# openhumanoids/pronto

Measured on NVIDIA B200. Metric: rbis_ekf_filter_steps_per_s, higher is better.
Workload: dtype f64

## Files before the change

### dev/kbench.cu

```cuda
#include <cuda_runtime.h>
#include <cmath>
#include <cstdio>
#include <cstdlib>
#include <cstring>
#include <vector>
#include <string>

#define CK(x) do { cudaError_t e = (x); if (e != cudaSuccess) { printf("CUDA error %s at %s:%d\n", cudaGetErrorString(e), __FILE__, __LINE__); exit(1); } } while (0)

struct Variant {
  const char* name;
  int tpb;
  int smem;
  void (*geom)(long long N, int sms, int* grid, int* tpb, int* smem);
  void (*launch)(void* kparams_blob, int grid, int tpb, int smem, cudaStream_t st);
  size_t kparams_size;
  void (*fill)(void* blob, long long N, double* vec, double* quat, double* P, double* ll, double* q4, const double* imu,
               const void* ops, long long n_ops, const double* z0, const double* z1, const double* q1, const double* R0,
               const double* R1);
  void (*prep)(int smem);
};
std::vector<Variant>& registry() { static std::vector<Variant> r; return r; }

__global__ void __launch_bounds__(256) dfma_probe(double* out, int iters, double a, int active_lanes) {
// ... 89 lines not shown
        double v = (i == j) ? 0.01 * (1 + 0.1 * rnd()) : 1e-4 * rnd();
        if (decoupled && (passive(i) || passive(j)) && !blk) v = 0.0;
        P[(size_t)(j * (j + 1) / 2 + i) * N + n] = v;
      }
    q4[n] = 7.6e-5; q4[N + n] = 1e-2; q4[2 * N + n] = 3e-10; q4[3 * N + n] = 1e-6;
    for (int i = 0; i < pi; i++) for (int c = 0; c < 4; c++) q1[((size_t)i * 4 + c) * N + n] = quat[c * N + n];
  }
  for (auto& v : imu) v = 0.05 * rnd();
  for (long long k = 0; k < T; k++) for (long long n = 0; n < N; n++) imu[(k * 6 + 5) * N + n] += 9.8;
  for (auto& v : z0) v = 0.1 * rnd();
  for (auto& v : z1) v = 0.1 * rnd();
  double R0[9] = {0.01, 0, 0, 0, 0.01, 0, 0, 0, 0.01};
  double R1[36] = {0};
  for (int i = 0; i < 6; i++) R1[i * 7] = i < 3 ? 0.0025 : 0.0012;
  double *d_vec, *d_quat, *d_P, *d_ll, *d_q4, *d_imu, *d_z0, *d_z1, *d_q1, *d_R0, *d_R1;
  void* d_ops;
  CK(cudaMalloc(&d_vec, vec.size() * 8)); CK(cudaMalloc(&d_quat, quat.size() * 8)); CK(cudaMalloc(&d_P, P.size() * 8));
  CK(cudaMalloc(&d_ll, N * 8)); CK(cudaMalloc(&d_q4, q4.size() * 8)); CK(cudaMalloc(&d_imu, imu.size() * 8));
  CK(cudaMalloc(&d_z0, z0.size() * 8)); CK(cudaMalloc(&d_z1, z1.size() * 8)); CK(cudaMalloc(&d_q1, q1.size() * 8));
  CK(cudaMalloc(&d_R0, 81 * 8)); CK(cudaMalloc(&d_R1, 81 * 8)); CK(cudaMalloc(&d_ops, ops.size() * sizeof(Op)));
  CK(cudaMemcpy(d_q4, q4.data(), q4.size() * 8, cudaMemcpyHostToDevice));
  CK(cudaMemcpy(d_imu, imu.data(), imu.size() * 8, cudaMemcpyHostToDevice));
  CK(cudaMemcpy(d_z0, z0.data(), z0.size() * 8, cudaMemcpyHostToDevice));
  CK(cudaMemcpy(d_z1, z1.data(), z1.size() * 8, cudaMemcpyHostToDevice));
  CK(cudaMemcpy(d_q1, q1.data(), q1.size() * 8, cudaMemcpyHostToDevice));
  CK(cudaMemcpy(d_R0, R0, 72, cudaMemcpyHostToDevice)); CK(cudaMemcpy(d_R1, R1, 36 * 8, cudaMemcpyHostToDevice));
  CK(cudaMemcpy(d_ops, ops.data(), ops.size() * sizeof(Op), cudaMemcpyHostToDevice));
  std::vector<double> ref_vec, ref_P, out_vec(vec.size()), out_P(P.size());
  for (auto& v : registry()) {
    if (only && !strstr(v.name, only)) continue;
    std::vector<char> blob(v.kparams_size, 0);
    int grid, tpb, smem;
    v.geom(N, prop.multiProcessorCount, &grid, &tpb, &smem);
    v.prep(smem);
    float best = 1e30f;
    for (int rep = 0; rep < 3; rep++) {
      CK(cudaMemcpy(d_vec, vec.data(), vec.size() * 8, cudaMemcpyHostToDevice));
      CK(cudaMemcpy(d_quat, quat.data(), quat.size() * 8, cudaMemcpyHostToDevice));
      CK(cudaMemcpy(d_P, P.data(), P.size() * 8, cudaMemcpyHostToDevice));
      CK(cudaMemset(d_ll, 0, N * 8));
      v.fill(blob.data(), N, d_vec, d_quat, d_P, d_ll, d_q4, d_imu, d_ops, (long long)ops.size(), d_z0, d_z1, d_q1, d_R0, d_R1);
      CK(cudaEventRecord(e0));
      v.launch(blob.data(), grid, tpb, smem, 0);
      CK(cudaEventRecord(e1)); CK(cudaEventSynchronize(e1)); CK(cudaGetLastError());
      CK(cudaEventElapsedTime(&ms, e0, e1));
      if (ms < best) best = ms;
    }
    CK(cudaMemcpy(out_vec.data(), d_vec, vec.size() * 8, cudaMemcpyDeviceToHost));
    CK(cudaMemcpy(out_P.data(), d_P, P.size() * 8, cudaMemcpyDeviceToHost));
    double ev = 0, eP = 0;
    if (ref_vec.empty()) { ref_vec = out_vec; ref_P = out_P; }
    for (size_t i = 0; i < out_vec.size(); i++) ev = fmax(ev, fabs(out_vec[i] - ref_vec[i]) / fmax(1.0, fabs(ref_vec[i])));
    for (size_t i = 0; i < out_P.size(); i++) eP = fmax(eP, fabs(out_P[i] - ref_P[i]) / 0.01);
    bool finite = true;
    for (size_t i = 0; i < out_vec.size(); i++) if (!std::isfinite(out_vec[i])) finite = false;
    printf("%-28s grid %4d x %3d thr, %6d B smem: %8.3f ms  %7.3f G filter-steps/s  (vs first: dvec %.2e dP %.2e finite=%d)\n", v.name, grid, tpb, smem, best,
// ... 5 lines not shown
```

### dev/kvariant.cu

```cuda
#include <cuda_runtime.h>
#include <cstring>
#include <vector>
#define rbisk VNAME
#ifdef KV1
#define KFUNC rbis_fused_kernel
#define SET_FAST(s, c, v)
#else
#ifdef KGROUP
#ifndef KDC
#define KDC 0
#endif
#ifndef KMAXW
#define KMAXW 8
#endif
#define KFUNC grp::rbis_group_kernel<KGROUP, (KDC != 0), KMAXW>
#elif defined(KDC)
#define KFUNC rbis_fused_kernel<false, true>
#else
#define KFUNC rbis_fused_kernel<false>
#endif
#define SET_FAST(s, c, v) s.chunk_fast[c] = v
#endif
#ifndef KHEADER
#define KHEADER "../pronto_b200/csrc/rbis_kernels.cuh"
// ... 35 lines not shown
  *smem = wpc * GE::FPW * GE::S * 8;
}
#else
void geom(long long N, int, int* grid, int* tpb, int* smem) {
  *tpb = VNAME::TPB; *smem = VNAME::SMEM_BYTES; *grid = (int)((N + VNAME::TPB - 1) / VNAME::TPB);
}
#endif
void prep(int smem) { cudaFuncSetAttribute(VNAME::KFUNC, cudaFuncAttributeMaxDynamicSharedMemorySize, smem); }
void fill(void* blob, long long N, double* vec, double* quat, double* P, double* ll, double* q4, const double* imu,
          const void* ops, long long n_ops, const double* z0, const double* z1, const double* q1, const double* R0,
          const double* R1) {
  VNAME::KParams kp;
  std::memset(&kp, 0, sizeof(kp));
  kp.N = N; kp.vec = vec; kp.quat = quat; kp.P = P; kp.loglik = ll;
  kp.q_gyro = q4; kp.q_accel = q4 + N; kp.q_gyro_bias = q4 + 2 * N; kp.q_accel_bias = q4 + 3 * N;
  kp.imu = imu; kp.imu_cols = N; kp.ops = (const VNAME::Op*)ops; kp.n_ops = n_ops; kp.g_val = 9.8; kp.chi_tol = 1e-6; kp.ctor_folds_chi = 1;
  auto& s0 = kp.streams[0];
  s0.m = 3; s0.has_orient = 0; s0.r_mode = 0; s0.n_chunks = 1; s0.idx[0] = 3; s0.idx[1] = 4; s0.idx[2] = 5;
  s0.chunk_start[0] = 0; s0.chunk_len[0] = 3; SET_FAST(s0, 0, 3); s0.z = z0; s0.R = R0; s0.cols = N;
  auto& s1 = kp.streams[1];
  s1.m = 6; s1.has_orient = 1; s1.r_mode = 0; s1.n_chunks = 2;
  int idx[6] = {9, 10, 11, 6, 7, 8};
  for (int i = 0; i < 6; i++) s1.idx[i] = idx[i];
  s1.chunk_start[0] = 0; s1.chunk_len[0] = 3; s1.chunk_start[1] = 3; s1.chunk_len[1] = 3; SET_FAST(s1, 0, 9); SET_FAST(s1, 1, 6); s1.z = z1; s1.quat = q1; s1.R = R1; s1.cols = N;
  std::memcpy(blob, &kp, sizeof(kp));
}
struct Reg { Reg() { registry().push_back({VTAG, VNAME::TPB, VNAME::SMEM_BYTES, geom, launch, sizeof(VNAME::KParams), fill, prep}); } } reg;
}
```

### include/rbis_batch.h

```cpp
#ifndef RBIS_BATCH_H_
#define RBIS_BATCH_H_

#include <stdint.h>

#ifdef __cplusplus
extern "C" {
#endif

#define RBIS_NUM_STATES 21
#define RBIS_COV_ELEMS 441
#define RBIS_MAX_MEAS 9
#define RBIS_MAX_STREAMS 8
#define RBIS_NUM_STATS 96

typedef struct rbis_batch rbis_batch_t;

typedef enum {
  RBIS_OK = 0,
  RBIS_ERR_INVALID = -1,
  RBIS_ERR_CUDA = -2,
  RBIS_ERR_ALLOC = -3,
  RBIS_ERR_STATE = -4
} rbis_status_t;

// ... 96 lines not shown
  int32_t cov_blocks;
} rbis_record_t;
int rbis_batch_set_record(rbis_batch_t* h, const rbis_record_t* rec);

#define RBIS_INNOV_NIS    1
#define RBIS_INNOV_Y      2
#define RBIS_INNOV_S_DIAG 4
typedef struct {
  uint32_t fields;
  int32_t  m;
  double*  out;
  int64_t  rows;
} rbis_innovation_t;
int rbis_batch_set_innovations(rbis_batch_t* h, int32_t stream, const rbis_innovation_t* spec);

int rbis_batch_run_fused(rbis_batch_t* h, int64_t n_ops, const rbis_op_t* ops, const double* imu,
                         int64_t imu_rows, int n_streams, const rbis_stream_t* streams, int mem);

typedef struct {
  int32_t m;
  int32_t has_orientation;
  int32_t channel;
  int32_t channel_rot;
  const double* mean;
  const double* mean_quat;
  const int64_t* step;
  double sigma[RBIS_MAX_MEAS];
  double sigma_rot[3];
  int64_t rows;
} rbis_synth_stream_t;
typedef struct {
  uint64_t seed;
// ... 114 lines not shown
```

### pronto_b200/capi.py

```python
import ctypes as C
import os

_HERE = os.path.dirname(os.path.abspath(__file__))
LIB_PATH = os.path.join(_HERE, "lib", "librbis_b200.so")

NUM_STATES = 21
COV_ELEMS = 441
MAX_MEAS = 9
MAX_STREAMS = 8
NUM_STATS = 96

MEM_HOST, MEM_DEVICE = 0, 1
MEM_F32_ROWS = 4
OP_IMU, OP_MEAS, OP_SNAPSHOT, OP_RESTORE, OP_RECORD = 0, 1, 2, 3, 4
REC_FIELDS = 47
REC_BLOCKS = 7
INNOV_NIS, INNOV_Y, INNOV_S_DIAG = 1, 2, 4
R_SHARED_FULL, R_PER_FILTER_DIAG, R_PER_ROW_FULL = 0, 1, 2
STREAM_SKIP_NAN_ROWS = 1

c_double_p = C.POINTER(C.c_double)
c_int32_p = C.POINTER(C.c_int32)
c_int64_p = C.POINTER(C.c_int64)


class Config(C.Structure):
    _fields_ = [
        ("g_val", C.c_double),
        ("chi_tol", C.c_double),
# ... 106 lines not shown
    ]


PROTOTYPES = {
    "rbis_last_error": (C.c_char_p, []),
    "rbis_default_config": (None, [C.POINTER(Config)]),
    "rbis_batch_create": (C.c_int, [C.POINTER(C.c_void_p), C.c_int64, C.POINTER(Config)]),
    "rbis_batch_destroy": (C.c_int, [C.c_void_p]),
    "rbis_batch_synchronize": (C.c_int, [C.c_void_p]),
    "rbis_batch_num_filters": (C.c_int64, [C.c_void_p]),
    "rbis_batch_stream": (C.c_void_p, [C.c_void_p]),
    "rbis_batch_launch_count": (C.c_int64, [C.c_void_p]),
    "rbis_batch_last_kernel_variant": (C.c_int, [C.c_void_p]),
    "rbis_batch_notch_configure": (C.c_int, [C.c_void_p, C.c_double, C.c_double, C.c_int, C.c_int64]),
    "rbis_batch_notch_filter": (C.c_int, [C.c_void_p, C.c_void_p, C.c_int64, C.c_int]),
    "rbis_smooth_plan": (C.c_int64, [C.c_int64, C.c_void_p, C.c_void_p, C.c_void_p, C.c_void_p, C.c_void_p, C.c_void_p]),
    "rbis_batch_smooth_backward": (C.c_int, [C.c_void_p, C.c_int32, C.c_int32, C.c_int64, C.c_void_p, C.c_double]),
    "rbis_batch_get_snapshot": (C.c_int, [C.c_void_p, C.c_int32, C.c_void_p, C.c_void_p, C.c_void_p, C.c_void_p, C.c_int]),
    "rbis_batch_set_state": (C.c_int, [C.c_void_p, C.c_void_p, C.c_void_p, C.c_void_p, C.c_void_p, C.c_int64, C.c_int]),
    "rbis_batch_get_state": (C.c_int, [C.c_void_p, C.c_void_p, C.c_void_p, C.c_void_p, C.c_void_p, c_int64_p, C.c_int]),
    "rbis_batch_set_filter": (C.c_int, [C.c_void_p, C.c_int64, C.c_void_p, C.c_void_p, C.c_void_p, C.c_double]),
    "rbis_batch_get_filter": (C.c_int, [C.c_void_p, C.c_int64, C.c_void_p, C.c_void_p, C.c_void_p, c_double_p]),
    "rbis_batch_set_process_noise": (C.c_int, [C.c_void_p, C.c_double, C.c_double, C.c_double, C.c_double]),
    "rbis_batch_set_process_noise_per_filter": (C.c_int, [C.c_void_p, C.c_void_p, C.c_void_p, C.c_void_p, C.c_void_p, C.c_int]),
    "rbis_batch_ins_step": (C.c_int, [C.c_void_p, C.c_void_p, C.c_void_p, C.c_double, C.c_int64, C.c_int]),
    "rbis_batch_indexed_update": (C.c_int, [C.c_void_p, C.c_int, c_int32_p, C.c_void_p, C.c_void_p, C.c_int, C.c_int64, C.c_int]),
    "rbis_batch_indexed_orient_update": (C.c_int, [C.c_void_p, C.c_int, c_int32_p, C.c_void_p, C.c_void_p, C.c_void_p, C.c_int, C.c_int64, C.c_int]),
    "rbis_batch_set_column_map": (C.c_int, [C.c_void_p, C.c_int, C.c_void_p, C.c_int64]),
    "rbis_batch_set_record": (C.c_int, [C.c_void_p, C.POINTER(Record)]),
    "rbis_batch_set_innovations": (C.c_int, [C.c_void_p, C.c_int32, C.POINTER(Innovation)]),
# ... 65 lines not shown
```

### pronto_b200/csrc/rbis_batch.cu

```cuda
#include <cuda_runtime.h>
#include <dlfcn.h>

#include <algorithm>
#include <cmath>
#include <cstdarg>
#include <cstdio>
#include <cstring>
#include <new>
#include <string>
#include <vector>

#include "../../include/rbis_batch.h"
#include "rbis_kernels.cuh"
#include "rbis_stats.cuh"
#include "rbis_smooth.cuh"
#include "rbis_synth.cuh"
#include "rbis_fused_tu.h"

namespace {

thread_local std::string g_last_error;

int fail(int code, const char* fmt, ...) {
  char buf[512];
// ... 71 lines not shown
  int* d_flag = nullptr;
  rbisk::NotchCoeffs notch{};
  double* d_notch_state = nullptr;
  int64_t notch_cols = 0;
  DevBuf notch_stage;
  int last_variant = -1;
  int mapping = 1;
  int lane_tpb = 384;
  int n_sms = 148;
  long long last_part = -1;
  DevBuf full_cov;
  DevBuf misc;
  DevBuf stats_async;
  DevBuf synth_small;
  DevBuf stats_table;
  rbisk::Op* d_ops = nullptr;
  size_t d_ops_cap = 0;
  double* d_rshared = nullptr;
  StagingSlot slots[2];
  int slot_toggle = 0;
  int* d_map[1 + RBIS_MAX_STREAMS] = {};
  int64_t map_cols[1 + RBIS_MAX_STREAMS] = {};
  static constexpr int kMaxGroups = 8, kRing = 8;
  int n_groups = 1;
  cudaStream_t gstream[kMaxGroups] = {};
  cudaStream_t upload_stream = nullptr;
  cudaEvent_t gdone[kRing][kMaxGroups] = {};
  bool gdone_valid[kRing] = {};
  cudaEvent_t uploaded[kRing] = {};
  cudaEvent_t pre_evt = nullptr;
  cudaEvent_t syn_evt = nullptr;
  static constexpr int kPinSlots = 16;
  static constexpr size_t kPinBytes = 128 << 10;
  char* pin_base = nullptr;
  cudaEvent_t pin_evt[kPinSlots] = {};
  int pin_next = 0;
  DevBuf d_syn;
  DevBuf d_syn_ring[kRing];
  rbisk::Op* d_ops_ring[kRing] = {};
  size_t d_ops_ring_cap[kRing] = {};
  double* d_rshared_ring[kRing] = {};
  int64_t launch_seq = 0;
  int last_ring = -1;
  bool groups_dirty = false;
  bool stream_dirty = true;
  cudaEvent_t tickets[8] = {};
  int next_ticket = 0;
  bool rec_set = false;
  rbis_record_t rec{};
  int rec_k = 0;
  cudaStream_t rec_stream = nullptr;
  cudaEvent_t rec_launched = nullptr;
  DevBuf rec_stage[2];
  cudaEvent_t rec_copied[2] = {};
  bool rec_pending[2] = {};
// ... 177 lines not shown
  auto aligned_triple = [&](int a) {
    return d.idx[a] % 3 == 0 && d.idx[a + 1] == d.idx[a] + 1 && d.idx[a + 2] == d.idx[a] + 2;
  };
  for (size_t i = 0; i + 1 < cut.size();) {
    const int a = cut[i], blen = cut[i + 1] - cut[i];
    if (blen == 1 && i + 3 < cut.size() && cut[i + 2] - cut[i + 1] == 1 && cut[i + 3] - cut[i + 2] == 1 && aligned_triple(a)) {
      d.chunk_start[d.n_chunks] = a;
      d.chunk_len[d.n_chunks++] = 3;
      i += 3;
      continue;
    }
    d.chunk_start[d.n_chunks] = a;
    d.chunk_len[d.n_chunks++] = blen;
    i += 1;
  }
}

int upload_small(rbis_batch* h, void* dst, const void* src, size_t bytes, cudaStream_t st) {
  if (bytes == 0) return 0;
  if (!h->pin_base || bytes > rbis_batch::kPinBytes) {
    CUDA_TRY(cudaMemcpyAsync(dst, src, bytes, cudaMemcpyHostToDevice, st));
    return 0;
  }
  const int k = h->pin_next;
  h->pin_next = (k + 1) % rbis_batch::kPinSlots;
  CUDA_TRY(cudaEventSynchronize(h->pin_evt[k]));
  char* p = h->pin_base + (size_t)k * rbis_batch::kPinBytes;
  std::memcpy(p, src, bytes);
  CUDA_TRY(cudaMemcpyAsync(dst, p, bytes, cudaMemcpyHostToDevice, st));
  CUDA_TRY(cudaEventRecord(h->pin_evt[k], st));
// ... 218 lines not shown
      case RBIS_OP_RESTORE:
        if (o.row < 0 || o.row >= h->cfg.snapshot_slots) return fail(RBIS_ERR_INVALID, "op %lld: snapshot slot %lld out of range (%d slots)", (long long)i, (long long)o.row, h->cfg.snapshot_slots);
        if (!snap_valid[(size_t)o.row]) return fail(RBIS_ERR_STATE, "op %lld: restore of empty snapshot slot %lld", (long long)i, (long long)o.row);
        if (!snap_dc[(size_t)o.row]) restores_ok = false;
        last_utime = o.utime;
        break;
      case RBIS_OP_RECORD:
        if (!h->rec_set) return fail(RBIS_ERR_STATE, "op %lld: RBIS_OP_RECORD but no record set (rbis_batch_set_record)", (long long)i);
        if (o.row < 0 || o.row >= h->rec.rows) return fail(RBIS_ERR_INVALID, "op %lld: record row %lld out of range (%lld rows)", (long long)i, (long long)o.row, (long long)h->rec.rows);
        rec_rows.push_back(o.row);
        any_record = true;
        break;
      default:
        return fail(RBIS_ERR_INVALID, "op %lld: unknown kind %d", (long long)i, o.kind);
    }
  }

  rbisk::KParams kp;
  std::memset(&kp, 0, sizeof(kp));
  kp.N = N;
  kp.vec = h->vec; kp.quat = h->quat; kp.P = h->P; kp.loglik = h->loglik;
  kp.q_gyro = h->qparams; kp.q_accel = h->qparams + N; kp.q_gyro_bias = h->qparams + 2 * N;
  kp.q_accel_bias = h->qparams + 3 * N;
  kp.snap = h->snap;
  kp.n_snap = h->cfg.snapshot_slots;
  kp.n_ops = n_ops;
  kp.g_val = h->cfg.g_val; kp.chi_tol = h->cfg.chi_tol;
  kp.ctor_folds_chi = h->cfg.ctor_folds_chi; kp.renorm = h->cfg.renormalize_quat;

  kp.imu_map = use_maps ? h->d_map[0] : nullptr;
// ... 229 lines not shown
  if (any_snapshot && !h->snap_read_pending.empty()) {
    for (int64_t i = 0; i < n_ops; i++)
      if (ops[i].kind == RBIS_OP_SNAPSHOT && h->snap_read_pending[(size_t)ops[i].row]) {
        slot_readers.push_back(h->snap_read_evt[(size_t)ops[i].row]);
        h->snap_read_pending[(size_t)ops[i].row] = 0;
      }
  }
  if (any_record && !rec_host) take_readers(h, h->rec.out, h->rec.out + (size_t)h->rec.rows * (size_t)h->rec_k * N, slot_readers);
  for (int s = 0; s < n_streams; s++)
    if (innov_used[s]) take_readers(h, h->innov[s].out, h->innov[s].out + (size_t)h->innov[s].rows * (size_t)h->innov_k[s] * N, slot_readers);
  if (!grouped) {
    if (int rc = main_stream_work(h)) return rc;
    for (cudaEvent_t e : slot_readers) CUDA_TRY(cudaStreamWaitEvent(h->stream, e, 0));
    if (staging) CUDA_TRY(cudaStreamWaitEvent(h->stream, slot.copied, 0));
    if (rec_host && h->rec_pending[rec_b]) CUDA_TRY(cudaStreamWaitEvent(h->stream, h->rec_copied[rec_b], 0));
    if ((size_t)n_ops > h->d_ops_cap) {
      if (h->d_ops) {
        CUDA_TRY(cudaStreamSynchronize(h->stream));
        cudaFree(h->d_ops);
        h->d_ops = nullptr;
        h->d_ops_cap = 0;
      }
      size_t cap = (size_t)n_ops * 2;
      if (cap < 1024) cap = 1024;
      CUDA_TRY(cudaMalloc(&h->d_ops, cap * sizeof(rbisk::Op)));
      h->d_ops_cap = cap;
    }
    if (int rc = upload_small(h, h->d_ops, kops.data(), (size_t)n_ops * sizeof(rbisk::Op), h->stream)) return rc;
    if (any_shared)
      if (int rc = upload_small(h, h->d_rshared, rshared.data(), rshared.size() * sizeof(double), h->stream)) return rc;
    if (fuse_syn) {
      if (h->d_syn.cap < syn_host.size()) {
        CUDA_TRY(cudaStreamSynchronize(h->stream));
        if (h->d_syn.ensure(syn_host.size() * 2)) return fail(RBIS_ERR_ALLOC, "synth row buffer allocation failed");
      }
      if (int rc = upload_small(h, h->d_syn.p, syn_host.data(), syn_host.size() * 8, h->stream)) return rc;
      point_syn(h->d_syn.p);
    }
    kp.ops = h->d_ops;
    kp.block_offset = 0;
    CUDA_TRY(launch_variant(variant, fuse_syn ? 1 : 0, geom, grid, h->stream, kp));
    h->launches++;
    if (staging) CUDA_TRY(cudaEventRecord(slot.consumed, h->stream));
    if (rec_host) {
      CUDA_TRY(cudaEventRecord(h->rec_launched, h->stream));
      CUDA_TRY(cudaStreamWaitEvent(h->rec_stream, h->rec_launched, 0));
    }
  } else {
    const int64_t piece_ops = h->cfg.piece_ops > 0 ? h->cfg.piece_ops : 256;
    const int64_t pieces = n_ops >= 2 * piece_ops ? (n_ops + piece_ops - 1) / piece_ops : 1;
    const unsigned per = (grid + (unsigned)h->n_groups - 1) / (unsigned)h->n_groups;
    const long long part = (long long)per * geom.fpc;
    for (int64_t pc = 0; pc < pieces; pc++) {
      const int64_t o0 = n_ops * pc / pieces, o1 = n_ops * (pc + 1) / pieces, np = o1 - o0;
      const int ring = (int)(h->launch_seq % rbis_batch::kRing);
      if (h->gdone_valid[ring])
        for (int g = 0; g < h->n_groups; g++) CUDA_TRY(cudaEventSynchronize(h->gdone[ring][g]));
      if ((size_t)np > h->d_ops_ring_cap[ring]) {
        if (h->d_ops_ring[ring]) cudaFree(h->d_ops_ring[ring]);
        h->d_ops_ring[ring] = nullptr;
        h->d_ops_ring_cap[ring] = 0;
        size_t cap = (size_t)np * 2;
        if (cap < 1024) cap = 1024;
        CUDA_TRY(cudaMalloc(&h->d_ops_ring[ring], cap * sizeof(rbisk::Op)));
        h->d_ops_ring_cap[ring] = cap;
      }
      if (int rc = upload_small(h, h->d_ops_ring[ring], kops.data() + o0, (size_t)np * sizeof(rbisk::Op), h->upload_stream)) return rc;
      if (any_shared) {
        if (int rc = upload_small(h, h->d_rshared_ring[ring], rshared.data(), rshared.size() * sizeof(double), h->upload_stream)) return rc;
        for (int s2 = 0; s2 < n_streams; s2++)
          if (shared_r[s2]) kp.streams[s2].R = h->d_rshared_ring[ring] + (size_t)s2 * kRShared;
      }
      if (fuse_syn) {
        if (h->d_syn_ring[ring].cap < syn_host.size() && h->d_syn_ring[ring].ensure(syn_host.size() * 2))
          return fail(RBIS_ERR_ALLOC, "synth row buffer allocation failed");
        if (int rc = upload_small(h, h->d_syn_ring[ring].p, syn_host.data(), syn_host.size() * 8, h->upload_stream)) return rc;
        point_syn(h->d_syn_ring[ring].p);
      }
      CUDA_TRY(cudaEventRecord(h->uploaded[ring], h->upload_stream));
      kp.ops = h->d_ops_ring[ring];
      kp.n_ops = np;
      const bool wait_main = h->stream_dirty;
      if (wait_main) CUDA_TRY(cudaEventRecord(h->pre_evt, h->stream));
      const bool repartitioned = h->last_ring >= 0 && h->groups_dirty && h->last_part != part;
      for (int g = 0; g < h->n_groups; g++) {
        const unsigned b0 = (unsigned)g * per, b1 = b0 + per < grid ? b0 + per : grid;
        cudaStream_t gs = h->gstream[g];
        if (repartitioned)
          for (int g2 = 0; g2 < h->n_groups; g2++) CUDA_TRY(cudaStreamWaitEvent(gs, h->gdone[h->last_ring][g2], 0));
        if (wait_main) CUDA_TRY(cudaStreamWaitEvent(gs, h->pre_evt, 0));
        if (pc == 0)
          for (cudaEvent_t e : slot_readers) CUDA_TRY(cudaStreamWaitEvent(gs, e, 0));
        if (staging && pc == 0) CUDA_TRY(cudaStreamWaitEvent(gs, slot.copied, 0));
        if (rec_host && pc == 0 && h->rec_pending[rec_b]) CUDA_TRY(cudaStreamWaitEvent(gs, h->rec_copied[rec_b], 0));
        CUDA_TRY(cudaStreamWaitEvent(gs, h->uploaded[ring], 0));
        if (b1 > b0) {
          kp.block_offset = (int)b0;
          CUDA_TRY(launch_variant(variant, fuse_syn ? 1 : 0, geom, b1 - b0, gs, kp));
          h->launches++;
        }
        CUDA_TRY(cudaEventRecord(h->gdone[ring][g], gs));
      }
      h->gdone_valid[ring] = true;
      h->last_ring = ring;
      h->last_part = part;
      h->groups_dirty = true;
      h->stream_dirty = false;
      if (staging) slot.ring = ring;
      if (pc + 1 < pieces) h->launch_seq++;
    }
    if (rec_host)
      for (int g = 0; g < h->n_groups; g++) CUDA_TRY(cudaStreamWaitEvent(h->rec_stream, h->gdone[h->last_ring][g], 0));
  }
  if (rec_host) {
    const size_t row_doubles = (size_t)h->rec_k * (size_t)N;
    for (size_t a = 0; a < rec_distinct.size();) {
      size_t e = a + 1;
      while (e < rec_distinct.size() && rec_distinct[e] == rec_distinct[e - 1] + 1) e++;
      CUDA_TRY(cudaMemcpyAsync(h->rec.out + (size_t)rec_distinct[a] * row_doubles, h->rec_stage[rec_b].p + a * row_doubles,
                               (e - a) * row_doubles * sizeof(double), cudaMemcpyDeviceToHost, h->rec_stream));
      a = e;
    }
    CUDA_TRY(cudaEventRecord(h->rec_copied[rec_b], h->rec_stream));
    h->rec_pending[rec_b] = true;
// ... 10 lines not shown
    const char as_launch = ((variant & 2) || (before == 1 && !passive_index && restores_ok)) ? 1 : 0;
    for (auto& f : snap_dc)
      if (f == 2) f = as_launch;
  }
  h->snap_dc = snap_dc;
  h->last_variant = variant | (fuse_syn ? 4 : 0) | (h->mapping > 1 ? (h->mapping << 4) : 0);
  h->utime = last_utime;
  return 0;
}

}

extern "C" {

const char* rbis_last_error(void) { return g_last_error.c_str(); }

void rbis_default_config(rbis_batch_config_t* cfg) {
  if (!cfg) return;
  cfg->g_val = 9.8;
  cfg->chi_tol = 1e-6;
  cfg->ctor_folds_chi = 1;
  cfg->renormalize_quat = 0;
  cfg->snapshot_slots = 0;
  cfg->device = 0;
  cfg->launch_groups = 0;
  cfg->dense_only = 0;
  cfg->mapping = 0;
  cfg->lane_filters_per_cta = 0;
  cfg->piece_ops = 0;
  cfg->synth_materialize = 0;
// ... 118 lines not shown
  if (h->copy_stream) cudaStreamSynchronize(h->copy_stream);
  if (h->rec_stream) { cudaStreamSynchronize(h->rec_stream); cudaStreamDestroy(h->rec_stream); }
  if (h->rec_launched) cudaEventDestroy(h->rec_launched);
  for (auto& e : h->rec_copied)
    if (e) cudaEventDestroy(e);
  for (auto& e : h->ticket_rec)
    if (e) cudaEventDestroy(e);
  for (auto& b : h->rec_stage) b.release();
  if (h->upload_stream) { cudaStreamSynchronize(h->upload_stream); cudaStreamDestroy(h->upload_stream); }
  for (int g = 0; g < rbis_batch::kMaxGroups; g++)
    if (h->gstream[g]) { cudaStreamSynchronize(h->gstream[g]); cudaStreamDestroy(h->gstream[g]); }
  for (int r = 0; r < rbis_batch::kRing; r++) {
    if (h->uploaded[r]) cudaEventDestroy(h->uploaded[r]);
    for (int g = 0; g < rbis_batch::kMaxGroups; g++)
      if (h->gdone[r][g]) cudaEventDestroy(h->gdone[r][g]);
    cudaFree(h->d_ops_ring[r]);
    cudaFree(h->d_rshared_ring[r]);
  }
  if (h->pre_evt) cudaEventDestroy(h->pre_evt);
  if (h->syn_evt) cudaEventDestroy(h->syn_evt);
  for (auto& e : h->pin_evt)
    if (e) cudaEventDestroy(e);
  if (h->pin_base) cudaFreeHost(h->pin_base);
  cudaFree(h->vec); cudaFree(h->quat); cudaFree(h->P); cudaFree(h->loglik); cudaFree(h->qparams);
  cudaFree(h->snap); cudaFree(h->d_ops); cudaFree(h->d_rshared); cudaFree(h->d_flag); cudaFree(h->d_notch_state);
  h->notch_stage.release();
  for (auto& m : h->d_map) cudaFree(m);
  h->full_cov.release(); h->misc.release(); h->stats_async.release(); h->stats_table.release(); h->synth_small.release(); h->d_syn.release();
  for (auto& b : h->snap_stats_scratch) b.release();
  for (cudaEvent_t e : h->snap_read_evt) if (e) cudaEventDestroy(e);
  for (auto& r : h->row_readers) cudaEventDestroy(r.done);
  if (h->rec_stats_done) cudaEventDestroy(h->rec_stats_done);
  h->rec_stats_scratch.release();
  if (h->stats_stream) cudaStreamDestroy(h->stats_stream);
  for (auto& b : h->d_syn_ring) b.release();
  for (auto& s : h->slots) {
    s.imu.release(); s.f32.release(); s.rtab.release();
    for (int i = 0; i < RBIS_MAX_STREAMS; i++) { s.z[i].release(); s.quat[i].release(); s.rdiag[i].release(); }
    if (s.copied) cudaEventDestroy(s.copied);
    if (s.consumed) cudaEventDestroy(s.consumed);
// ... 822 lines not shown
```

### pronto_b200/csrc/rbis_group.cuh

```cuda
#ifndef RBIS_GROUP_CUH_
#define RBIS_GROUP_CUH_

namespace rbisk {
namespace grp {

template <int G, bool DC>
struct Geo {
  static_assert(G == 2 || G == 4 || G == 8 || G == 16, "lanes per filter");
  static constexpr int NA = DC ? N_ACT : NS;
  static constexpr int LD = NA;
  static constexpr int FPW = 32 / G;
  static constexpr int NJ = (NA + G - 1) / G;
  static constexpr int stride_() {
    int s = NA * LD;
    while (s % 16 != G % 16) s++;
    return s;
  }
  static constexpr int S = stride_();
  static constexpr int PV = DC ? 0 : 3, PC = DC ? 3 : 6, PP = DC ? 6 : 9, PG = DC ? 9 : 15, PA = DC ? 12 : 18;
};
template <bool DC>
__device__ __forceinline__ int pos_of(int idx) { return DC ? (idx < 12 ? idx - 3 : idx - 6) : idx; }
template <bool DC>
__host__ __device__ constexpr int idx_of(int pos) { return DC ? act_col(pos) : pos; }
// ... 550 lines not shown
  const int wpc = blockDim.x >> 5;
  const long long N = p.N;
  long long n = (((long long)blockIdx.x + p.block_offset) * wpc + warp) * FPW + lane / G;
  const bool active = n < N;
  if (!active) n = N - 1;
  const bool writer = active && l == 0;
  double* Pf = smem + (size_t)(warp * FPW + lane / G) * S;

  FilterState s;
  static_for<NS>([&](auto i) { s.x[i] = p.vec[(long long)i * N + n]; });
  s.qw = p.quat[n]; s.qx = p.quat[N + n]; s.qy = p.quat[2 * N + n]; s.qz = p.quat[3 * N + n];
  s.ll = p.loglik[n];
  g_cov_load<G, DC>(Pf, l, p.P + n, N);
  bool imu_seen = false;

  auto load_op = [&](long long i) {
    Op o;
    long long w0, w1;
    asm volatile("ld.global.nc.s64 %0, [%1];" : "=l"(w0) : "l"(reinterpret_cast<const long long*>(p.ops + i)));
    asm volatile("ld.global.nc.s64 %0, [%1];" : "=l"(w1) : "l"(reinterpret_cast<const long long*>(p.ops + i) + 1));
    o.kind = (int)(w0 & 0xffffffffll); o.stream = (int)(w0 >> 32); o.row = w1;
    asm volatile("ld.global.nc.f64 %0, [%1];" : "=d"(o.dt) : "l"(&p.ops[i].dt));
    return o;
  };
  const long long imu_n = p.imu_map ? (long long)__ldg(p.imu_map + n) : n;
  QNoise qn;
  qn.q_gyro = __ldg(p.q_gyro + n); qn.q_accel = __ldg(p.q_accel + n);
  qn.q_gyro_bias = __ldg(p.q_gyro_bias + n); qn.q_accel_bias = __ldg(p.q_accel_bias + n);

  auto prefetch = [&](const double* ptr) { asm volatile("prefetch.global.L1 [%0];" ::"l"(ptr)); };
  unsigned long long syn_kf = 0;
  double syn_sg = 0.0, syn_sa = 0.0;
  if constexpr (SYN) {
    syn_kf = p.syn.seed ^ ((unsigned long long)(p.syn.first_filter + n) * SYN_K1);
    syn_sg = p.syn.sigma_gyro >= 0 ? p.syn.sigma_gyro : sqrt(__ldg(p.q_gyro + n) / p.syn.dt);
    syn_sa = p.syn.sigma_accel >= 0 ? p.syn.sigma_accel : sqrt(__ldg(p.q_accel + n) / p.syn.dt);
  }
  auto prefetch_inputs = [&](const Op& o) {
    if (o.kind == OP_IMU) {
      const double* base = p.imu + o.row * 6 * p.imu_cols + imu_n;
#pragma unroll
      for (int k = 0; k < 6; k++) prefetch(base + k * p.imu_cols);
    } else if (o.kind == OP_MEAS) {
      const StreamDesc& st = p.streams[o.stream];
      const long long sn = st.map ? (long long)__ldg(st.map + n) : n;
      const double* zb = st.z + o.row * st.m * st.cols + sn;
      for (int a = 0; a < st.m; a++) prefetch(zb + a * st.cols);
      if (st.has_orient) {
        const double* qb = st.quat + o.row * 4 * st.cols + sn;
#pragma unroll
        for (int k = 0; k < 4; k++) prefetch(qb + k * st.cols);
      }
    }
  };
  Op op1 = load_op(0);
  Op op2 = p.n_ops > 1 ? load_op(1) : op1;
  for (long long oi = 0; oi < p.n_ops; oi++) {
    const Op op = op1;
    op1 = op2;
    if (oi + 2 < p.n_ops) op2 = load_op(oi + 2);
    if constexpr (!SYN) {
      if (oi + 1 < p.n_ops) prefetch_inputs(op1);
    }
    if (op.kind == OP_IMU) {
      const double* base = p.imu + op.row * 6 * p.imu_cols + imu_n;
      const long long Ni = p.imu_cols;
      V3 gyro, acc;
      if constexpr (SYN) {
        const unsigned long long kfs = syn_kf ^ ((unsigned long long)__ldg(p.syn.imu_step + op.row) * SYN_K2);
        const double* mu = p.syn.imu_mean + op.row * 6;
        double nn[6];
        syn_normals_k<1, 6>(kfs, 0u, nn);
        gyro = {fma(syn_sg, nn[0], __ldg(mu)), fma(syn_sg, nn[1], __ldg(mu + 1)), fma(syn_sg, nn[2], __ldg(mu + 2))};
        acc = {fma(syn_sa, nn[3], __ldg(mu + 3)), fma(syn_sa, nn[4], __ldg(mu + 4)), fma(syn_sa, nn[5], __ldg(mu + 5))};
      } else {
        gyro = {ldg_early(base), ldg_early(base + Ni), ldg_early(base + 2 * Ni)};
        acc = {ldg_early(base + 3 * Ni), ldg_early(base + 4 * Ni), ldg_early(base + 5 * Ni)};
// ... 127 lines not shown
```

### pronto_b200/csrc/rbis_kernels.cuh

```cuda
#if defined(rbisk) || !defined(RBIS_KERNELS_CUH_DEFAULT)
#ifndef rbisk
#define RBIS_KERNELS_CUH_DEFAULT
#endif
#include <cstdint>
#include <utility>

#define RBIS_SCHED_FENCE() asm volatile("" ::: "memory")
#ifndef RBIS_LATE_LOADS
#define RBIS_LATE_LOADS 0
#endif
#ifndef RBIS_PARK_STATE
#define RBIS_PARK_STATE 0
#endif

namespace rbisk {

constexpr int NS = 21;
constexpr int NP = 231;
#ifndef RBIS_TPB
#define RBIS_TPB 256
#endif
constexpr int TPB = RBIS_TPB;
constexpr int SWEEP_TILE = 8;
constexpr int MAX_MEAS = 9;
// ... 96 lines not shown
  int chunk_fast[MAX_CHUNKS];
  const double* z;
  const double* quat;
  const double* R;
  const int* map;
  long long cols;
  long long r_stride;
};

struct Op {
  int kind, stream;
  long long row;
  double dt;
};
constexpr int OP_IMU = 0, OP_MEAS = 1, OP_SNAPSHOT = 2, OP_RECORD = 4;

constexpr unsigned long long SYN_K1 = 0x9E3779B97F4A7C15ull, SYN_K2 = 0xC2B2AE3D27D4EB4Full, SYN_K3 = 0x165667B19E3779F9ull;
__host__ __device__ __forceinline__ unsigned long long splitmix64(unsigned long long x) {
  x += 0x9E3779B97F4A7C15ull;
  x = (x ^ (x >> 30)) * 0xBF58476D1CE4E5B9ull;
  x = (x ^ (x >> 27)) * 0x94D049BB133111EBull;
  return x ^ (x >> 31);
}
struct SynPair {
  float r, th;
};
__device__ __forceinline__ SynPair syn_pair_k(unsigned long long kfs, unsigned even_channel) {
  const unsigned long long a = splitmix64(kfs ^ ((unsigned long long)even_channel * SYN_K3));
  const float u1 = ((float)(unsigned)(a >> 40) + 0.5f) * (1.0f / 16777216.0f);
  const float u2 = (float)((unsigned)(a >> 16) & 0xffffffu) * (1.0f / 16777216.0f);
// ... 83 lines not shown

struct KParams {
  long long N;
  double* vec;
  double* quat;
  double* P;
  double* loglik;
  const double* q_gyro;
  const double* q_accel;
  const double* q_gyro_bias;
  const double* q_accel_bias;
  const double* imu;
  const int* imu_map;
  long long imu_cols;
  double* snap;
  const Op* ops;
  long long n_ops;
  double g_val, chi_tol;
  int ctor_folds_chi, renorm, n_snap;
  int block_offset;
  StreamDesc streams[MAX_STREAMS];
  SynK syn;
  RecK rec;
  unsigned skip_nan_streams;
  unsigned rec_cov_blocks;
  InnovK innov[MAX_STREAMS];
};

template <int... Is, class F>
__device__ __forceinline__ void static_for_impl(std::integer_sequence<int, Is...>, F&& f) {
  (f(std::integral_constant<int, Is>{}), ...);
}
template <int N, class F>
__device__ __forceinline__ void static_for(F&& f) {
  static_for_impl(std::make_integer_sequence<int, N>{}, static_cast<F&&>(f));
}

struct V3 {
  double x, y, z;
};
__device__ __forceinline__ V3 cross(const V3& a, const V3& b) {
  return {fma(a.y, b.z, -(a.z * b.y)), fma(a.z, b.x, -(a.x * b.z)), fma(a.x, b.y, -(a.y * b.x))};
// ... 1000 lines not shown
  long long n = ((long long)blockIdx.x + p.block_offset) * TPB + tid;
  const bool active = n < N;
  if (!active) n = N - 1;

  Cov P;
  P.Ps = smem + tid;
  P.tm = tm_base + ((uint32_t)((warp & 3) * 32) << 16) + (uint32_t)((warp >> 2) * TM_COLS);
  FilterState s;
  static_for<NS>([&](auto i) { s.x[i] = p.vec[(long long)i * N + n]; });
  s.qw = p.quat[n]; s.qx = p.quat[N + n]; s.qy = p.quat[2 * N + n]; s.qz = p.quat[3 * N + n];
  s.ll = p.loglik[n];
  if constexpr (DC) cov_load_active(P, p.P + n, N);
  else cov_load_all(P, p.P + n, N);
  bool imu_seen = false;

  auto load_op = [&](long long i) {
    Op o;
    long long w0, w1;
    asm volatile("ld.global.nc.s64 %0, [%1];" : "=l"(w0) : "l"(reinterpret_cast<const long long*>(p.ops + i)));
    asm volatile("ld.global.nc.s64 %0, [%1];" : "=l"(w1) : "l"(reinterpret_cast<const long long*>(p.ops + i) + 1));
    o.kind = (int)(w0 & 0xffffffffll); o.stream = (int)(w0 >> 32); o.row = w1;
    asm volatile("ld.global.nc.f64 %0, [%1];" : "=d"(o.dt) : "l"(&p.ops[i].dt));
    return o;
  };
  const long long imu_n = p.imu_map ? (long long)__ldg(p.imu_map + n) : n;
  unsigned long long syn_kf = 0;
  double syn_sg = 0.0, syn_sa = 0.0;
  if constexpr (SYN) {
    syn_kf = p.syn.seed ^ ((unsigned long long)(p.syn.first_filter + n) * SYN_K1);
    syn_sg = p.syn.sigma_gyro >= 0 ? p.syn.sigma_gyro : sqrt(__ldg(p.q_gyro + n) / p.syn.dt);
    syn_sa = p.syn.sigma_accel >= 0 ? p.syn.sigma_accel : sqrt(__ldg(p.q_accel + n) / p.syn.dt);
  }
  Op op_next = load_op(0);
  for (long long oi = 0; oi < p.n_ops; oi++) {
    const Op op = op_next;
    if (oi + 1 < p.n_ops) op_next = load_op(oi + 1);
    if (op.kind == OP_IMU) {
      const double* base = p.imu + op.row * 6 * p.imu_cols + imu_n;
      const long long Ni = p.imu_cols;
      V3 gyro, acc;
      QNoise qn;
      auto load_q = [&]() {
        qn.q_gyro = ldg_early(p.q_gyro + n); qn.q_accel = ldg_early(p.q_accel + n);
        qn.q_gyro_bias = ldg_early(p.q_gyro_bias + n); qn.q_accel_bias = ldg_early(p.q_accel_bias + n);
      };
      auto load_inputs = [&]() {
        if constexpr (SYN) {
          const unsigned long long kfs = syn_kf ^ ((unsigned long long)__ldg(p.syn.imu_step + op.row) * SYN_K2);
          const double* mu = p.syn.imu_mean + op.row * 6;
          double nn[6];
          syn_normals_k<1, 6>(kfs, 0u, nn);
// ... 198 lines not shown
```

Baseline: 7.238 billion.

## Pass the op schedule as a packed table in kernel parameters instead of global memory

```diff
diff --git a/dev/kbench.cu b/dev/kbench.cu
--- a/dev/kbench.cu
+++ b/dev/kbench.cu
@@ -127,18 +127,16 @@
   double R1[36] = {0};
   for (int i = 0; i < 6; i++) R1[i * 7] = i < 3 ? 0.0025 : 0.0012;
   double *d_vec, *d_quat, *d_P, *d_ll, *d_q4, *d_imu, *d_z0, *d_z1, *d_q1, *d_R0, *d_R1;
-  void* d_ops;
   CK(cudaMalloc(&d_vec, vec.size() * 8)); CK(cudaMalloc(&d_quat, quat.size() * 8)); CK(cudaMalloc(&d_P, P.size() * 8));
   CK(cudaMalloc(&d_ll, N * 8)); CK(cudaMalloc(&d_q4, q4.size() * 8)); CK(cudaMalloc(&d_imu, imu.size() * 8));
   CK(cudaMalloc(&d_z0, z0.size() * 8)); CK(cudaMalloc(&d_z1, z1.size() * 8)); CK(cudaMalloc(&d_q1, q1.size() * 8));
-  CK(cudaMalloc(&d_R0, 81 * 8)); CK(cudaMalloc(&d_R1, 81 * 8)); CK(cudaMalloc(&d_ops, ops.size() * sizeof(Op)));
+  CK(cudaMalloc(&d_R0, 81 * 8)); CK(cudaMalloc(&d_R1, 81 * 8));
   CK(cudaMemcpy(d_q4, q4.data(), q4.size() * 8, cudaMemcpyHostToDevice));
   CK(cudaMemcpy(d_imu, imu.data(), imu.size() * 8, cudaMemcpyHostToDevice));
   CK(cudaMemcpy(d_z0, z0.data(), z0.size() * 8, cudaMemcpyHostToDevice));
   CK(cudaMemcpy(d_z1, z1.data(), z1.size() * 8, cudaMemcpyHostToDevice));
   CK(cudaMemcpy(d_q1, q1.data(), q1.size() * 8, cudaMemcpyHostToDevice));
   CK(cudaMemcpy(d_R0, R0, 72, cudaMemcpyHostToDevice)); CK(cudaMemcpy(d_R1, R1, 36 * 8, cudaMemcpyHostToDevice));
-  CK(cudaMemcpy(d_ops, ops.data(), ops.size() * sizeof(Op), cudaMemcpyHostToDevice));
   std::vector<double> ref_vec, ref_P, out_vec(vec.size()), out_P(P.size());
   for (auto& v : registry()) {
     if (only && !strstr(v.name, only)) continue;
@@ -152,7 +150,7 @@
       CK(cudaMemcpy(d_quat, quat.data(), quat.size() * 8, cudaMemcpyHostToDevice));
       CK(cudaMemcpy(d_P, P.data(), P.size() * 8, cudaMemcpyHostToDevice));
       CK(cudaMemset(d_ll, 0, N * 8));
-      v.fill(blob.data(), N, d_vec, d_quat, d_P, d_ll, d_q4, d_imu, d_ops, (long long)ops.size(), d_z0, d_z1, d_q1, d_R0, d_R1);
+      v.fill(blob.data(), N, d_vec, d_quat, d_P, d_ll, d_q4, d_imu, ops.data(), (long long)ops.size(), d_z0, d_z1, d_q1, d_R0, d_R1);
       CK(cudaEventRecord(e0));
       v.launch(blob.data(), grid, tpb, smem, 0);
       CK(cudaEventRecord(e1)); CK(cudaEventSynchronize(e1)); CK(cudaGetLastError());
diff --git a/dev/kvariant.cu b/dev/kvariant.cu
--- a/dev/kvariant.cu
+++ b/dev/kvariant.cu
@@ -73,7 +73,20 @@
   std::memset(&kp, 0, sizeof(kp));
   kp.N = N; kp.vec = vec; kp.quat = quat; kp.P = P; kp.loglik = ll;
   kp.q_gyro = q4; kp.q_accel = q4 + N; kp.q_gyro_bias = q4 + 2 * N; kp.q_accel_bias = q4 + 3 * N;
-  kp.imu = imu; kp.imu_cols = N; kp.ops = (const VNAME::Op*)ops; kp.n_ops = n_ops; kp.g_val = 9.8; kp.chi_tol = 1e-6; kp.ctor_folds_chi = 1;
+  kp.imu = imu; kp.imu_cols = N; kp.g_val = 9.8; kp.chi_tol = 1e-6; kp.ctor_folds_chi = 1;
+  const VNAME::Op* o = (const VNAME::Op*)ops;
+  int nd = 0;
+  long long i = 0;
+  for (; i < n_ops && i < VNAME::OPTAB_OPS; i++) {
+    int di = 0;
+    while (di < nd && std::memcmp(&kp.prog.dt[di], &o[i].dt, 8)) di++;
+    if (di == nd) {
+      if (nd == VNAME::OPTAB_DTS) break;
+      kp.prog.dt[nd++] = o[i].dt;
+    }
+    kp.prog.op[i] = VNAME::optab_word(o[i].kind, o[i].stream, (unsigned)di, (unsigned long long)o[i].row);
+  }
+  kp.n_ops = i;
   auto& s0 = kp.streams[0];
   s0.m = 3; s0.has_orient = 0; s0.r_mode = 0; s0.n_chunks = 1; s0.idx[0] = 3; s0.idx[1] = 4; s0.idx[2] = 5;
   s0.chunk_start[0] = 0; s0.chunk_len[0] = 3; SET_FAST(s0, 0, 3); s0.z = z0; s0.R = R0; s0.cols = N;
diff --git a/include/rbis_batch.h b/include/rbis_batch.h
--- a/include/rbis_batch.h
+++ b/include/rbis_batch.h
@@ -134,8 +134,11 @@
 } rbis_innovation_t;
 int rbis_batch_set_innovations(rbis_batch_t* h, int32_t stream, const rbis_innovation_t* spec);
 
+#define RBIS_OP_TABLE_OPS 1024
+#define RBIS_OP_TABLE_DTS 256
 int rbis_batch_run_fused(rbis_batch_t* h, int64_t n_ops, const rbis_op_t* ops, const double* imu,
                          int64_t imu_rows, int n_streams, const rbis_stream_t* streams, int mem);
+int64_t rbis_op_table_encode(const rbis_op_t* ops, int64_t n_ops, uint64_t* words, double* dts, int32_t* n_dts);
 
 typedef struct {
   int32_t m;
diff --git a/pronto_b200/capi.py b/pronto_b200/capi.py
--- a/pronto_b200/capi.py
+++ b/pronto_b200/capi.py
@@ -13,6 +13,7 @@
 MEM_HOST, MEM_DEVICE = 0, 1
 MEM_F32_ROWS = 4
 OP_IMU, OP_MEAS, OP_SNAPSHOT, OP_RESTORE, OP_RECORD = 0, 1, 2, 3, 4
+OP_TABLE_OPS, OP_TABLE_DTS = 1024, 256
 REC_FIELDS = 47
 REC_BLOCKS = 7
 INNOV_NIS, INNOV_Y, INNOV_S_DIAG = 1, 2, 4
@@ -149,6 +150,7 @@
     "rbis_batch_last_kernel_variant": (C.c_int, [C.c_void_p]),
     "rbis_batch_notch_configure": (C.c_int, [C.c_void_p, C.c_double, C.c_double, C.c_int, C.c_int64]),
     "rbis_batch_notch_filter": (C.c_int, [C.c_void_p, C.c_void_p, C.c_int64, C.c_int]),
+    "rbis_op_table_encode": (C.c_int64, [C.c_void_p, C.c_int64, C.c_void_p, C.c_void_p, C.c_void_p]),
     "rbis_smooth_plan": (C.c_int64, [C.c_int64, C.c_void_p, C.c_void_p, C.c_void_p, C.c_void_p, C.c_void_p, C.c_void_p]),
     "rbis_batch_smooth_backward": (C.c_int, [C.c_void_p, C.c_int32, C.c_int32, C.c_int64, C.c_void_p, C.c_double]),
     "rbis_batch_get_snapshot": (C.c_int, [C.c_void_p, C.c_int32, C.c_void_p, C.c_void_p, C.c_void_p, C.c_void_p, C.c_int]),
diff --git a/pronto_b200/csrc/rbis_batch.cu b/pronto_b200/csrc/rbis_batch.cu
--- a/pronto_b200/csrc/rbis_batch.cu
+++ b/pronto_b200/csrc/rbis_batch.cu
@@ -109,8 +109,6 @@
   DevBuf stats_async;
   DevBuf synth_small;
   DevBuf stats_table;
-  rbisk::Op* d_ops = nullptr;
-  size_t d_ops_cap = 0;
   double* d_rshared = nullptr;
   StagingSlot slots[2];
   int slot_toggle = 0;
@@ -132,8 +130,6 @@
   int pin_next = 0;
   DevBuf d_syn;
   DevBuf d_syn_ring[kRing];
-  rbisk::Op* d_ops_ring[kRing] = {};
-  size_t d_ops_ring_cap[kRing] = {};
   double* d_rshared_ring[kRing] = {};
   int64_t launch_seq = 0;
   int last_ring = -1;
@@ -341,6 +337,32 @@
     d.chunk_len[d.n_chunks++] = blen;
     i += 1;
   }
+}
+
+static_assert(RBIS_OP_TABLE_OPS == rbisk::OPTAB_OPS && RBIS_OP_TABLE_DTS == rbisk::OPTAB_DTS, "op table capacity");
+int64_t optab_fill(const rbisk::Op* ops, int64_t n, rbisk::OpTab* t) {
+  int n_dt = 0, last = 0;
+  int64_t i = 0;
+  for (; i < n && i < rbisk::OPTAB_OPS; i++) {
+    const rbisk::Op& o = ops[i];
+    int di = 0;
+    if (o.kind == RBIS_OP_IMU) {
+      auto same = [&](int k) { return std::memcmp(&t->dt[k], &o.dt, sizeof(double)) == 0; };
+      if (n_dt > 0 && same(last)) {
+        di = last;
+      } else {
+        di = 0;
+        while (di < n_dt && !same(di)) di++;
+        if (di == n_dt) {
+          if (n_dt == rbisk::OPTAB_DTS) break;
+          t->dt[n_dt++] = o.dt;
+        }
+        last = di;
+      }
+    }
+    t->op[i] = rbisk::optab_word(o.kind, o.kind == RBIS_OP_MEAS ? o.stream : 0, (unsigned)di, (unsigned long long)o.row);
+  }
+  return i;
 }
 
 int upload_small(rbis_batch* h, void* dst, const void* src, size_t bytes, cudaStream_t st) {
@@ -589,6 +611,7 @@
       default:
         return fail(RBIS_ERR_INVALID, "op %lld: unknown kind %d", (long long)i, o.kind);
     }
+    if (o.row > (int64_t)0xffffffffll) return fail(RBIS_ERR_INVALID, "op %lld: row %lld does not fit the op table's 32 bits", (long long)i, (long long)o.row);
   }
 
   rbisk::KParams kp;
@@ -848,19 +871,6 @@
     for (cudaEvent_t e : slot_readers) CUDA_TRY(cudaStreamWaitEvent(h->stream, e, 0));
     if (staging) CUDA_TRY(cudaStreamWaitEvent(h->stream, slot.copied, 0));
     if (rec_host && h->rec_pending[rec_b]) CUDA_TRY(cudaStreamWaitEvent(h->stream, h->rec_copied[rec_b], 0));
-    if ((size_t)n_ops > h->d_ops_cap) {
-      if (h->d_ops) {
-        CUDA_TRY(cudaStreamSynchronize(h->stream));
-        cudaFree(h->d_ops);
-        h->d_ops = nullptr;
-        h->d_ops_cap = 0;
-      }
-      size_t cap = (size_t)n_ops * 2;
-      if (cap < 1024) cap = 1024;
-      CUDA_TRY(cudaMalloc(&h->d_ops, cap * sizeof(rbisk::Op)));
-      h->d_ops_cap = cap;
-    }
-    if (int rc = upload_small(h, h->d_ops, kops.data(), (size_t)n_ops * sizeof(rbisk::Op), h->stream)) return rc;
     if (any_shared)
       if (int rc = upload_small(h, h->d_rshared, rshared.data(), rshared.size() * sizeof(double), h->stream)) return rc;
     if (fuse_syn) {
@@ -871,10 +881,14 @@
       if (int rc = upload_small(h, h->d_syn.p, syn_host.data(), syn_host.size() * 8, h->stream)) return rc;
       point_syn(h->d_syn.p);
     }
-    kp.ops = h->d_ops;
     kp.block_offset = 0;
-    CUDA_TRY(launch_variant(variant, fuse_syn ? 1 : 0, geom, grid, h->stream, kp));
-    h->launches++;
+    for (int64_t o0 = 0; o0 < n_ops;) {
+      const int64_t np = optab_fill(kops.data() + o0, n_ops - o0, &kp.prog);
+      kp.n_ops = np;
+      CUDA_TRY(launch_variant(variant, fuse_syn ? 1 : 0, geom, grid, h->stream, kp));
+      h->launches++;
+      o0 += np;
+    }
     if (staging) CUDA_TRY(cudaEventRecord(slot.consumed, h->stream));
     if (rec_host) {
       CUDA_TRY(cudaEventRecord(h->rec_launched, h->stream));
@@ -883,23 +897,18 @@
   } else {
     const int64_t piece_ops = h->cfg.piece_ops > 0 ? h->cfg.piece_ops : 256;
     const int64_t pieces = n_ops >= 2 * piece_ops ? (n_ops + piece_ops - 1) / piece_ops : 1;
+    std::vector<int64_t> cuts{0};
+    for (int64_t pc = 0; pc < pieces; pc++) {
+      const int64_t o1 = n_ops * (pc + 1) / pieces;
+      while (cuts.back() < o1) cuts.push_back(cuts.back() + optab_fill(kops.data() + cuts.back(), o1 - cuts.back(), &kp.prog));
+    }
     const unsigned per = (grid + (unsigned)h->n_groups - 1) / (unsigned)h->n_groups;
     const long long part = (long long)per * geom.fpc;
-    for (int64_t pc = 0; pc < pieces; pc++) {
-      const int64_t o0 = n_ops * pc / pieces, o1 = n_ops * (pc + 1) / pieces, np = o1 - o0;
+    for (size_t pc = 0; pc + 1 < cuts.size(); pc++) {
+      const int64_t o0 = cuts[pc], np = cuts[pc + 1] - o0;
       const int ring = (int)(h->launch_seq % rbis_batch::kRing);
       if (h->gdone_valid[ring])
         for (int g = 0; g < h->n_groups; g++) CUDA_TRY(cudaEventSynchronize(h->gdone[ring][g]));
-      if ((size_t)np > h->d_ops_ring_cap[ring]) {
-        if (h->d_ops_ring[ring]) cudaFree(h->d_ops_ring[ring]);
-        h->d_ops_ring[ring] = nullptr;
-        h->d_ops_ring_cap[ring] = 0;
-        size_t cap = (size_t)np * 2;
-        if (cap < 1024) cap = 1024;
-        CUDA_TRY(cudaMalloc(&h->d_ops_ring[ring], cap * sizeof(rbisk::Op)));
-        h->d_ops_ring_cap[ring] = cap;
-      }
-      if (int rc = upload_small(h, h->d_ops_ring[ring], kops.data() + o0, (size_t)np * sizeof(rbisk::Op), h->upload_stream)) return rc;
       if (any_shared) {
         if (int rc = upload_small(h, h->d_rshared_ring[ring], rshared.data(), rshared.size() * sizeof(double), h->upload_stream)) return rc;
         for (int s2 = 0; s2 < n_streams; s2++)
@@ -912,7 +921,7 @@
         point_syn(h->d_syn_ring[ring].p);
       }
       CUDA_TRY(cudaEventRecord(h->uploaded[ring], h->upload_stream));
-      kp.ops = h->d_ops_ring[ring];
+      optab_fill(kops.data() + o0, np, &kp.prog);
       kp.n_ops = np;
       const bool wait_main = h->stream_dirty;
       if (wait_main) CUDA_TRY(cudaEventRecord(h->pre_evt, h->stream));
@@ -941,7 +950,7 @@
       h->groups_dirty = true;
       h->stream_dirty = false;
       if (staging) slot.ring = ring;
-      if (pc + 1 < pieces) h->launch_seq++;
+      if (pc + 2 < cuts.size()) h->launch_seq++;
     }
     if (rec_host)
       for (int g = 0; g < h->n_groups; g++) CUDA_TRY(cudaStreamWaitEvent(h->rec_stream, h->gdone[h->last_ring][g], 0));
@@ -982,6 +991,30 @@
 extern "C" {
 
 const char* rbis_last_error(void) { return g_last_error.c_str(); }
+
+int64_t rbis_op_table_encode(const rbis_op_t* ops, int64_t n_ops, uint64_t* words, double* dts, int32_t* n_dts) {
+  if (n_ops < 0 || (n_ops > 0 && !ops) || !words || !dts || !n_dts) return fail(RBIS_ERR_INVALID, "bad arguments");
+  const int64_t n = n_ops < rbisk::OPTAB_OPS ? n_ops : rbisk::OPTAB_OPS;
+  std::vector<rbisk::Op> kops((size_t)n);
+  for (int64_t i = 0; i < n; i++) {
+    const rbis_op_t& o = ops[i];
+    if (o.kind < RBIS_OP_IMU || o.kind > RBIS_OP_RECORD) return fail(RBIS_ERR_INVALID, "op %lld: unknown kind %d", (long long)i, o.kind);
+    if (o.row < 0 || o.row > (int64_t)0xffffffffll) return fail(RBIS_ERR_INVALID, "op %lld: row %lld does not fit the op table's 32 bits", (long long)i, (long long)o.row);
+    if (o.kind == RBIS_OP_MEAS && (o.stream < 0 || o.stream >= RBIS_MAX_STREAMS)) return fail(RBIS_ERR_INVALID, "op %lld: stream %d out of range", (long long)i, o.stream);
+    kops[(size_t)i] = {o.kind, o.stream, o.row, o.dt};
+  }
+  rbisk::OpTab t;
+  std::memset(&t, 0, sizeof(t));
+  const int64_t taken = optab_fill(kops.data(), n, &t);
+  int32_t nd = 0;
+  for (int64_t i = 0; i < taken; i++) {
+    words[i] = t.op[i];
+    if (kops[(size_t)i].kind == RBIS_OP_IMU) nd = std::max(nd, (int32_t)((t.op[i] >> 16) & 0xffffu) + 1);
+  }
+  std::memcpy(dts, t.dt, (size_t)nd * sizeof(double));
+  *n_dts = nd;
+  return taken;
+}
 
 void rbis_default_config(rbis_batch_config_t* cfg) {
   if (!cfg) return;
@@ -1130,7 +1163,6 @@
     if (h->uploaded[r]) cudaEventDestroy(h->uploaded[r]);
     for (int g = 0; g < rbis_batch::kMaxGroups; g++)
       if (h->gdone[r][g]) cudaEventDestroy(h->gdone[r][g]);
-    cudaFree(h->d_ops_ring[r]);
     cudaFree(h->d_rshared_ring[r]);
   }
   if (h->pre_evt) cudaEventDestroy(h->pre_evt);
@@ -1139,7 +1171,7 @@
     if (e) cudaEventDestroy(e);
   if (h->pin_base) cudaFreeHost(h->pin_base);
   cudaFree(h->vec); cudaFree(h->quat); cudaFree(h->P); cudaFree(h->loglik); cudaFree(h->qparams);
-  cudaFree(h->snap); cudaFree(h->d_ops); cudaFree(h->d_rshared); cudaFree(h->d_flag); cudaFree(h->d_notch_state);
+  cudaFree(h->snap); cudaFree(h->d_rshared); cudaFree(h->d_flag); cudaFree(h->d_notch_state);
   h->notch_stage.release();
   for (auto& m : h->d_map) cudaFree(m);
   h->full_cov.release(); h->misc.release(); h->stats_async.release(); h->stats_table.release(); h->synth_small.release(); h->d_syn.release();
diff --git a/pronto_b200/csrc/rbis_group.cuh b/pronto_b200/csrc/rbis_group.cuh
--- a/pronto_b200/csrc/rbis_group.cuh
+++ b/pronto_b200/csrc/rbis_group.cuh
@@ -588,15 +588,6 @@
   g_cov_load<G, DC>(Pf, l, p.P + n, N);
   bool imu_seen = false;
 
-  auto load_op = [&](long long i) {
-    Op o;
-    long long w0, w1;
-    asm volatile("ld.global.nc.s64 %0, [%1];" : "=l"(w0) : "l"(reinterpret_cast<const long long*>(p.ops + i)));
-    asm volatile("ld.global.nc.s64 %0, [%1];" : "=l"(w1) : "l"(reinterpret_cast<const long long*>(p.ops + i) + 1));
-    o.kind = (int)(w0 & 0xffffffffll); o.stream = (int)(w0 >> 32); o.row = w1;
-    asm volatile("ld.global.nc.f64 %0, [%1];" : "=d"(o.dt) : "l"(&p.ops[i].dt));
-    return o;
-  };
   const long long imu_n = p.imu_map ? (long long)__ldg(p.imu_map + n) : n;
   QNoise qn;
   qn.q_gyro = __ldg(p.q_gyro + n); qn.q_accel = __ldg(p.q_accel + n);
@@ -627,14 +618,11 @@
       }
     }
   };
-  Op op1 = load_op(0);
-  Op op2 = p.n_ops > 1 ? load_op(1) : op1;
-  for (long long oi = 0; oi < p.n_ops; oi++) {
-    const Op op = op1;
-    op1 = op2;
-    if (oi + 2 < p.n_ops) op2 = load_op(oi + 2);
+  const int n_ops = (int)p.n_ops;
+  for (int oi = 0; oi < n_ops; oi++) {
+    const Op op = optab_op(p.prog, oi);
     if constexpr (!SYN) {
-      if (oi + 1 < p.n_ops) prefetch_inputs(op1);
+      if (oi + 1 < n_ops) prefetch_inputs(optab_op(p.prog, oi + 1));
     }
     if (op.kind == OP_IMU) {
       const double* base = p.imu + op.row * 6 * p.imu_cols + imu_n;
diff --git a/pronto_b200/csrc/rbis_kernels.cuh b/pronto_b200/csrc/rbis_kernels.cuh
--- a/pronto_b200/csrc/rbis_kernels.cuh
+++ b/pronto_b200/csrc/rbis_kernels.cuh
@@ -134,6 +134,25 @@
   double dt;
 };
 constexpr int OP_IMU = 0, OP_MEAS = 1, OP_SNAPSHOT = 2, OP_RECORD = 4;
+
+constexpr int OPTAB_OPS = 1024;
+constexpr int OPTAB_DTS = 256;
+struct OpTab {
+  unsigned long long op[OPTAB_OPS];
+  double dt[OPTAB_DTS];
+};
+__host__ __device__ __forceinline__ unsigned long long optab_word(int kind, int stream, unsigned dt_index, unsigned long long row) {
+  return (unsigned long long)(unsigned)kind | ((unsigned long long)(unsigned)stream << 8) | ((unsigned long long)dt_index << 16) | (row << 32);
+}
+__host__ __device__ __forceinline__ Op optab_op(const OpTab& t, int i) {
+  const unsigned long long w = t.op[i];
+  Op o;
+  o.kind = (int)(w & 0xffu);
+  o.stream = (int)((w >> 8) & 0xffu);
+  o.row = (long long)(w >> 32);
+  o.dt = t.dt[(w >> 16) & 0xffffu];
+  return o;
+}
 
 constexpr unsigned long long SYN_K1 = 0x9E3779B97F4A7C15ull, SYN_K2 = 0xC2B2AE3D27D4EB4Full, SYN_K3 = 0x165667B19E3779F9ull;
 __host__ __device__ __forceinline__ unsigned long long splitmix64(unsigned long long x) {
@@ -247,7 +266,6 @@
   const int* imu_map;
   long long imu_cols;
   double* snap;
-  const Op* ops;
   long long n_ops;
   double g_val, chi_tol;
   int ctor_folds_chi, renorm, n_snap;
@@ -258,7 +276,9 @@
   unsigned skip_nan_streams;
   unsigned rec_cov_blocks;
   InnovK innov[MAX_STREAMS];
-};
+  OpTab prog;
+};
+static_assert(sizeof(KParams) <= 32764, "KParams exceeds the kernel parameter space");
 
 template <int... Is, class F>
 __device__ __forceinline__ void static_for_impl(std::integer_sequence<int, Is...>, F&& f) {
@@ -1289,15 +1309,6 @@
   else cov_load_all(P, p.P + n, N);
   bool imu_seen = false;
 
-  auto load_op = [&](long long i) {
-    Op o;
-    long long w0, w1;
-    asm volatile("ld.global.nc.s64 %0, [%1];" : "=l"(w0) : "l"(reinterpret_cast<const long long*>(p.ops + i)));
-    asm volatile("ld.global.nc.s64 %0, [%1];" : "=l"(w1) : "l"(reinterpret_cast<const long long*>(p.ops + i) + 1));
-    o.kind = (int)(w0 & 0xffffffffll); o.stream = (int)(w0 >> 32); o.row = w1;
-    asm volatile("ld.global.nc.f64 %0, [%1];" : "=d"(o.dt) : "l"(&p.ops[i].dt));
-    return o;
-  };
   const long long imu_n = p.imu_map ? (long long)__ldg(p.imu_map + n) : n;
   unsigned long long syn_kf = 0;
   double syn_sg = 0.0, syn_sa = 0.0;
@@ -1306,10 +1317,10 @@
     syn_sg = p.syn.sigma_gyro >= 0 ? p.syn.sigma_gyro : sqrt(__ldg(p.q_gyro + n) / p.syn.dt);
     syn_sa = p.syn.sigma_accel >= 0 ? p.syn.sigma_accel : sqrt(__ldg(p.q_accel + n) / p.syn.dt);
   }
-  Op op_next = load_op(0);
+  Op op_next = optab_op(p.prog, 0);
   for (long long oi = 0; oi < p.n_ops; oi++) {
     const Op op = op_next;
-    if (oi + 1 < p.n_ops) op_next = load_op(oi + 1);
+    if (oi + 1 < p.n_ops) op_next = optab_op(p.prog, (int)oi + 1);
     if (op.kind == OP_IMU) {
       const double* base = p.imu + op.row * 6 * p.imu_cols + imu_n;
       const long long Ni = p.imu_cols;
```

Result: no change. 7.181 billion (median of 6 runs) (-0.8%).
